# ethz-asl/laser_slam

Measured on AMD Instinct MI355X. Metric: scans_per_sec, higher is better.
Workload: dtype f32

## Files before the change

### laser_slam_amd/csrc/lsgpu_icp.hip

```cpp
#include <atomic>
#include <cstring>
#include <cmath>
#include <cstdio>
#include <cstdlib>
#include <string>
#include <vector>
#include <chrono>
#include <system_error>
#include <thread>
#include <type_traits>
#include <utility>

#include <dlfcn.h>

#include <hip/hip_runtime.h>
#include <rccl/rccl.h>

#include "../../include/lsgpu_icp.h"
#include "lsgpu_grid.hip.h"
#include "lsgpu_tuning.h"
#include "lsgpu_policy.h"
#include "lsgpu_knn.hip.h"
#include "lsgpu_knn_k.hip.h"
#include "lsgpu_snf.hip.h"
// ... 1781 lines not shown
      std::vector<uint32_t> sizes{(uint32_t)n}, next;
      h->gs_lvl_first.clear(); h->gs_lvl_blocks.clear();
      uint32_t rows = 0, segs = 0;
      for (int L = 0; L < glevels; ++L) {
        uint32_t fb = 0;
        next.clear();
        for (uint32_t c : sizes) {
          fb += (c + kGsTile - 1u) / kGsTile;
          next.push_back(c - c / 2u); next.push_back(c / 2u);
        }
        h->gs_lvl_first.push_back(rows); h->gs_lvl_blocks.push_back(fb);
        rows += fb; segs += (uint32_t)sizes.size();
        sizes.swap(next);
      }
      HIPC(h->gs_tab.reserve(rows)); HIPC(h->gs_sblk.reserve(segs));
      if (glevels <= kGsPlanLevels && ((size_t)1 << (glevels - 1)) <= kGsPlanSegs) {
        GsPlanArgs pa{};
        for (int L = 0; L < glevels; ++L) pa.first[L] = h->gs_lvl_first[L];
        hipLaunchKernelGGL(k_gs_plan, dim3(glevels), dim3(1024), 0, h->stream, (uint32_t)n, pa, h->gs_tab.p, h->gs_sblk.p);
        HIPC(hipGetLastError());
      } else {
        std::vector<GsBlock> tab;
        std::vector<GsSegBlocks> sblk;
        std::vector<std::pair<uint32_t, uint32_t>> segsz{{0u, (uint32_t)n}};
        for (int L = 0; L < glevels; ++L) {
          uint32_t fb = 0;
          std::vector<std::pair<uint32_t, uint32_t>> nx;
          for (uint32_t sidx = 0; sidx < segsz.size(); ++sidx) {
            const uint32_t st = segsz[sidx].first, c = segsz[sidx].second;
            const uint32_t nb = (c + kGsTile - 1u) / kGsTile;
            sblk.push_back(GsSegBlocks{fb, nb, st, c});
            for (uint32_t k = 0; k < nb; ++k)
              tab.push_back(GsBlock{st + k * kGsTile, std::min(kGsTile, c - k * kGsTile), sidx, st, c, fb, nb, 0u});
            fb += nb;
            const uint32_t left = c - c / 2u;
            nx.push_back({st, left}); nx.push_back({st + left, c - left});
          }
          segsz.swap(nx);
        }
        HIPC(hipMemcpyAsync(h->gs_tab.p, tab.data(), tab.size() * sizeof(GsBlock), hipMemcpyHostToDevice, h->stream));
        HIPC(hipMemcpyAsync(h->gs_sblk.p, sblk.data(), sblk.size() * sizeof(GsSegBlocks), hipMemcpyHostToDevice, h->stream));
        HIPC(hipStreamSynchronize(h->stream));
      }
      h->gs_plan_n = n; h->gs_plan_levels = glevels;
    }
    const size_t nseg_g = (size_t)1 << glevels;
    int cap = 1;
    for (uint32_t v : h->gs_lvl_blocks) cap = std::max(cap, (int)v);
    for (auto& bf : h->gs_e) HIPC(bf.reserve(n));
    for (auto& bf : h->gs_k) HIPC(bf.reserve(n));
    HIPC(h->gs_hist.reserve(4 * 256 * (nseg_g + 1))); HIPC(h->gs_median.reserve(nseg_g)); HIPC(h->gs_cand_n.reserve(2 * nseg_g + 2));
    const size_t cand_room = std::max<size_t>(nseg_g / 2, 1) * kGsCandRoom;
    HIPC(h->gs_cand.reserve(cand_room)); HIPC(h->gs_cand_blk.reserve(cand_room));
    HIPC(h->gs_cl.reserve((size_t)2 * cap)); HIPC(h->gs_err.reserve(8)); HIPC(h->gs_rng.reserve(2 * nseg_g + 2));
    HIPC(h->ssn_axis_a.reserve(nseg_g)); HIPC(h->ssn_axis_b.reserve(nseg_g));
    uint32_t* cand_n[2] = {h->gs_cand_n.p, h->gs_cand_n.p + nseg_g + 1};
    uint32_t* sig_cur = reinterpret_cast<uint32_t*>(h->ssn_axis_a.p);
    uint32_t* sig_nxt = reinterpret_cast<uint32_t*>(h->ssn_axis_b.p);
    GsSet in, out;
    in.e = h->gs_e[0].p; out.e = h->gs_e[1].p;
    for (int d = 0; d < 3; ++d) { in.k[d] = h->gs_k[d].p; out.k[d] = h->gs_k[3 + d].p; }
    uint2* rng_cur = h->gs_rng.p;
    uint2* rng_nxt = h->gs_rng.p + nseg_g + 1;
    uint32_t* gh1[2] = {h->gs_hist.p, h->gs_hist.p + 256 * (nseg_g + 1)};
    uint32_t* gh2[2] = {h->gs_hist.p + 2 * 256 * (nseg_g + 1), h->gs_hist.p + 3 * 256 * (nseg_g + 1)};
    hipLaunchKernelGGL(k_gs_init, dim3(nblk(n)), dim3(256), 0, h->stream, src, (int)n, in, out.e, (const SsnSeg*)cur, (const uint32_t*)h->ssn_bb.p, rng_cur,
                       gh1[0], gh2[0], cand_n[0], sig_cur, h->gs_err.p);
    for (int L = 0; L < glevels; ++L) {
      const int ns = 1 << L, nb = (int)h->gs_lvl_blocks[L], par = L & 1;
      const GsBlock* tab = h->gs_tab.p + h->gs_lvl_first[L];
      const GsSegBlocks* sblk = h->gs_sblk.p + (ns - 1);
      hipLaunchKernelGGL(k_gs_hist<1>, dim3(nb), dim3(256), 0, h->stream, tab, cur, (const uint2*)rng_cur, in, gh1[par], gh2[par], h->gs_err.p);
      hipLaunchKernelGGL(k_gs_hist<2>, dim3(nb), dim3(256), 0, h->stream, tab, cur, (const uint2*)rng_cur, in, gh1[par], gh2[par], h->gs_err.p);
      const uint32_t lvl_cap = (uint32_t)std::min<size_t>(cand_room / (size_t)ns, (size_t)1 << 22);
      hipLaunchKernelGGL(k_gs_collect, dim3(nb), dim3(256), 0, h->stream, tab, cur, (const uint2*)rng_cur, (const uint32_t*)sig_cur, in,
                         (const uint32_t*)gh1[par], (const uint32_t*)gh2[par], cand_n[par], h->gs_cand.p, h->gs_cand_blk.p, lvl_cap, h->gs_cl.p);
      hipLaunchKernelGGL(k_gs_select, dim3(ns), dim3(L < 3 ? 1024 : 256), 0, h->stream, sblk, src, cur, (const uint32_t*)sig_cur, gh1[par], gh2[par],
                         gh1[par ^ 1], gh2[par ^ 1], cand_n[par], (const GsMedian*)h->gs_cand.p, (const uint32_t*)h->gs_cand_blk.p, lvl_cap, h->gs_cl.p,
                         h->gs_cl.p + cap, h->gs_median.p, nxt, sig_nxt, cand_n[par ^ 1], rng_nxt, h->gs_err.p);
      hipLaunchKernelGGL(k_gs_part, dim3(nb), dim3(kGsPartThreads), 0, h->stream, tab, cur, (const uint32_t*)sig_cur, in, out,
                         (const GsMedian*)h->gs_median.p, (const uint32_t*)(h->gs_cl.p + cap), (const SsnSeg*)nxt, rng_nxt, h->gs_err.p);
      std::swap(in, out);
      std::swap(cur, nxt);
      std::swap(sig_cur, sig_nxt);
      std::swap(rng_cur, rng_nxt);
    }
    idx = in.e;
    root_sig = sig_cur;
    HIPC(hipGetLastError());
  } else if (glevels > 0) {
    const size_t nseg_g = (size_t)1 << glevels;
    const int cap = (int)(n / kSegTile + (int64_t)(nseg_g / 2) + 2);
    HIPC(h->lane.scratch->vals_alt.reserve(n));
    HIPC(h->ssn_axis_a.reserve(nseg_g)); HIPC(h->ssn_axis_b.reserve(nseg_g)); HIPC(h->ssn_seg_fb.reserve(nseg_g));
    HIPC(h->ssn_blocktab.reserve((size_t)cap)); HIPC(h->lane.scratch->sort_hist.reserve((size_t)256 * cap + 256 + 4));
    uint32_t* keyA = reinterpret_cast<uint32_t*>(h->lane.scratch->keys.p);
    uint32_t* keyB = keyA + n;
    uint32_t* valA = h->lane.scratch->vals.p;
    uint32_t* valB = h->lane.scratch->vals_alt.p;
    uint32_t* bh = h->lane.scratch->sort_hist.p;
    uint32_t* dtot = bh + (size_t)256 * cap;
    uint32_t* nblocks_dev = dtot + 256;
    int* ax_cur = h->ssn_axis_a.p;
    int* ax_nxt = h->ssn_axis_b.p;
    HIPC(hipMemsetAsync(ax_cur, 0xFF, sizeof(int), h->stream));
    for (int L = 0; L < glevels; ++L) {
      const int ns = 1 << L;
      const int grid = (int)std::min<int64_t>(cap, n / kSegTile + ns + 1);
      hipLaunchKernelGGL(k_ssn_plan, dim3(1), dim3(256), 0, h->stream, cur, ns, knn, ax_cur, h->ssn_seg_fb.p,
                         h->ssn_blocktab.p, nblocks_dev);
      hipLaunchKernelGGL(k_ssn_keys32, dim3(nblk(n)), dim3(256), 0, h->stream, src, (int)n, valA, h->ssn_seg_of.p, cur,
                         h->ssn_seg_fb.p, L == 0 ? 1 : 0, keyA);
      for (int pass = 0; pass < 4; ++pass) {
        const uint32_t* kin = (pass & 1) ? keyB : keyA; const uint32_t* vin = (pass & 1) ? valB : valA;
        uint32_t* kout = (pass & 1) ? keyA : keyB; uint32_t* vout = (pass & 1) ? valA : valB;
        hipLaunchKernelGGL(k_seg_hist<kSegItems>, dim3(grid), dim3(256), 0, h->stream, kin, h->ssn_blocktab.p, nblocks_dev, 8 * pass, bh, cap);
        hipLaunchKernelGGL(k_seg_scan, dim3(256), dim3(256), 0, h->stream, bh, cap, nblocks_dev, dtot);
        hipLaunchKernelGGL((k_seg_scatter<kSegItems>), dim3(grid), dim3(256), 0, h->stream, kin, vin, kout, vout,
                           h->ssn_blocktab.p, nblocks_dev, 8 * pass, bh, dtot, cap);
      }
      idx = valA;
      hipLaunchKernelGGL(k_ssn_split, dim3(nblk(ns)), dim3(256), 0, h->stream, src, idx, cur, ns, knn, nxt, (const int*)ax_cur, ax_nxt);
      hipLaunchKernelGGL(k_ssn_assign, dim3(nblk(n)), dim3(256), 0, h->stream, (int)n, cur, knn, h->ssn_seg_of.p, L == 0 ? 1 : 0);
      std::swap(cur, nxt);
      std::swap(ax_cur, ax_nxt);
    }
    root_axis = ax_cur;
    HIPC(hipGetLastError());
  }
  if (glevels < levels) {
    if (glevels == 0) {
      hipLaunchKernelGGL(k_ssn_keys, dim3(nblk(n)), dim3(256), 0, h->stream, src, (int)n, (const uint32_t*)nullptr,
                         (const uint32_t*)nullptr, cur, knn, h->lane.scratch->keys.p, h->lane.scratch->vals.p);
      idx = h->lane.scratch->vals.p;
    }
    uint32_t* idx_rw = const_cast<uint32_t*>(idx);
    if (root_max == 8192)
      hipLaunchKernelGGL(k_ssn_tree<8192>, dim3(1 << glevels), dim3(1024), 0, h->stream, src, idx_rw, cur, knn, levels - glevels, h->ssn_seg_of.p, nxt, root_axis, root_sig);
// ... 1793 lines not shown
```

### laser_slam_amd/csrc/lsgpu_ssn_select.hip.h

```cpp
#pragma once
#include "lsgpu_ssn.hip.h"
#include "lsgpu_ssn_tree.hip.h"

namespace lsgpu {

#ifdef LSGPU_KNN_STATS
#define LSGPU_SEL_T(n) do { if (gridDim.x == 1 && threadIdx.x == 0) g_tree_dbg[n] = (unsigned long long)clock64(); } while (0)
#else
#define LSGPU_SEL_T(n) do { } while (0)
#endif

constexpr uint32_t kGsTile = 2048u;
constexpr int kGsPartThreads = 512;
constexpr uint32_t kGsCandCap = 2048u;
constexpr uint32_t kGsCandRoom = 16384u;
constexpr uint32_t kGsNoAxis = 0xFFu;
constexpr uint32_t kGsSelBlocks = 8192u;

struct GsSet {
  uint32_t* e;
  uint32_t* k[3];
};
__device__ __forceinline__ uint32_t* gs_k(const GsSet& g, int d) { return d == 0 ? g.k[0] : d == 1 ? g.k[1] : g.k[2]; }

// ... 19 lines not shown
  if (o1 == a) { x1 = o2; x2 = o3; }
  else { x1 = o1; x2 = o2 == a ? o3 : o2; }
}
__device__ __forceinline__ bool gs_less(uint32_t ka, uint32_t k1, uint32_t k2, uint32_t e, const GsMedian& m) {
  return ka != m.ka ? ka < m.ka : k1 != m.k1 ? k1 < m.k1 : k2 != m.k2 ? k2 < m.k2 : e < m.e;
}

constexpr int kGsPlanLevels = 24;
constexpr uint32_t kGsPlanSegs = 8192u;
struct GsPlanArgs { uint32_t first[kGsPlanLevels]; };
__global__ __launch_bounds__(1024) void k_gs_plan(uint32_t n, GsPlanArgs lvl, GsBlock* __restrict__ tab, GsSegBlocks* __restrict__ sblk) {
  __shared__ uint32_t fbs[kGsPlanSegs + 1];
  __shared__ uint2 sc[kGsPlanSegs];
  __shared__ uint32_t wsum[16], carry_sh;
  const uint32_t L = blockIdx.x, ns = 1u << L;
  const int lane = threadIdx.x & 63, w = threadIdx.x >> 6;
  if (threadIdx.x == 0) carry_sh = 0u;
  __syncthreads();
  for (uint32_t s0 = 0; s0 < ns; s0 += 1024u) {
    const uint32_t sg = s0 + threadIdx.x;
    uint32_t st = 0u, c = n;
    for (int bit = (int)L - 1; bit >= 0; --bit) {
      const uint32_t left = c - c / 2u;
      if ((sg >> bit) & 1u) { st += left; c -= left; } else c = left;
    }
    const uint32_t nb = sg < ns ? (c + kGsTile - 1u) / kGsTile : 0u;
    const uint32_t incl = wave_scan_incl_u32(nb, lane);
    if (lane == 63) wsum[w] = incl;
    __syncthreads();
    uint32_t before = carry_sh;
    for (int ww = 0; ww < w; ++ww) before += wsum[ww];
    if (sg < ns) { fbs[sg] = before + incl - nb; sc[sg] = make_uint2(st, c); }
    __syncthreads();
    if (threadIdx.x == 1023) carry_sh = before + incl;
    __syncthreads();
  }
  if (threadIdx.x == 0) fbs[ns] = carry_sh;
  __syncthreads();
  const uint32_t total = fbs[ns];
  for (uint32_t sg = threadIdx.x; sg < ns; sg += 1024u)
    sblk[(ns - 1u) + sg] = GsSegBlocks{fbs[sg], fbs[sg + 1u] - fbs[sg], sc[sg].x, sc[sg].y};
  GsBlock* __restrict__ t = tab + lvl.first[L];
  for (uint32_t j = threadIdx.x; j < total; j += 1024u) {
    uint32_t lo = 0u, hi = ns;
    while (hi - lo > 1u) { const uint32_t mid = (lo + hi) >> 1; if (fbs[mid] <= j) lo = mid; else hi = mid; }
    const uint32_t k = j - fbs[lo], st = sc[lo].x, c = sc[lo].y;
    const uint32_t off = k * kGsTile;
    t[j] = GsBlock{st + off, min(kGsTile, c - off), lo, st, c, fbs[lo], fbs[lo + 1u] - fbs[lo], 0u};
  }
}

__global__ __launch_bounds__(256) void k_gs_init(const float4* __restrict__ p, int n, GsSet out, uint32_t* __restrict__ other_e,
                                                 const SsnSeg* __restrict__ root, const uint32_t* __restrict__ bb,
                                                 uint2* __restrict__ rng, uint32_t* __restrict__ gh1_root,
                                                 uint32_t* __restrict__ gh2_root, uint32_t* __restrict__ cand_n_root,
                                                 uint32_t* __restrict__ sig_root, uint32_t* __restrict__ err) {
  const int i = blockIdx.x * 256 + threadIdx.x;
  if (blockIdx.x == 0) {
    gh1_root[threadIdx.x] = 0u; gh2_root[threadIdx.x] = 0u;
    if (threadIdx.x < 8) err[threadIdx.x] = 0u;
    if (threadIdx.x == 0) {
      const int a = ssn_cut_axis(root[0]); rng[0] = make_uint2(bb[a], bb[3 + a]);
      cand_n_root[0] = 0u; sig_root[0] = 0xFFFFFFFFu;
    }
  }
  if (i >= n) return;
  const float4 v = p[i];
  out.e[i] = (uint32_t)i; other_e[i] = (uint32_t)i;
  out.k[0][i] = float_order_key(v.x); out.k[1][i] = float_order_key(v.y); out.k[2][i] = float_order_key(v.z);
}

struct GsCut { int a; uint32_t klo, khi; float xlo, scale; };
__device__ __forceinline__ GsCut gs_cut(const SsnSeg& sg, const uint2 rng ) {
  GsCut c;
  c.a = ssn_cut_axis(sg);
  c.klo = rng.x; c.khi = rng.y >= rng.x ? rng.y : rng.x;
  c.xlo = float_from_order_key(c.klo);
  const float ext = float_from_order_key(c.khi) - c.xlo;
  c.scale = ext > 0.f ? 65536.0f / ext : 0.f;
  return c;
}
__device__ __forceinline__ uint32_t gs_bin16(const GsCut& c, uint32_t k) {
  const float t = (float_from_order_key(k) - c.xlo) * c.scale;
  return (uint32_t)fminf(fmaxf(t, 0.f), 65535.f);
}

__device__ __forceinline__ void gs_find_bin(const uint32_t* __restrict__ gh, uint32_t target, uint32_t* sh ,
                                            uint32_t& bin, uint32_t& below) {
  const int lane = threadIdx.x & 63, w = threadIdx.x >> 6;
  const bool act = threadIdx.x < 256u;
  const uint32_t tot = act ? gh[threadIdx.x] : 0u;
  const uint32_t incl = wave_scan_incl_u32(tot, lane);
  if (threadIdx.x == 0) { sh[4] = 0xFFFFFFFFu; sh[5] = 0u; }
  if (act && lane == 63) sh[w] = incl;
  __syncthreads();
  uint32_t before = 0u;
  for (int ww = 0; ww < w && ww < 4; ++ww) before += sh[ww];
  const uint32_t excl = before + incl - tot;
  if (act && tot != 0u && excl <= target && target < excl + tot) { sh[4] = threadIdx.x; sh[5] = excl; }
  __syncthreads();
  bin = sh[4]; below = sh[5];
  __syncthreads();
}

template <int PASS>
__global__ __launch_bounds__(256) void k_gs_hist(const GsBlock* __restrict__ tab, const SsnSeg* __restrict__ segs,
                                                 const uint2* __restrict__ rng, GsSet in, uint32_t* __restrict__ gh1,
                                                 uint32_t* __restrict__ gh2, uint32_t* __restrict__ err) {
  __shared__ uint32_t hist[256];
  __shared__ uint32_t sh[8];
  hist[threadIdx.x] = 0u;
  const GsBlock sb = tab[blockIdx.x];
  const GsCut c = gs_cut(segs[sb.seg], rng[sb.seg]);
  const uint32_t* __restrict__ ka = gs_k(in, c.a);
  uint32_t mb1 = 0u, below1 = 0u;
// ... 22 lines not shown
                                                    uint32_t* __restrict__ cl) {
  __shared__ uint32_t ws[4];
  __shared__ uint32_t sh[8];
  const GsBlock sb = tab[blockIdx.x];
  const GsCut c = gs_cut(segs[sb.seg], rng[sb.seg]);
  const uint32_t leftn = sb.seg_count - sb.seg_count / 2u;
  uint32_t mb1, below1, mb2, below2;
  gs_find_bin(gh1 + (size_t)sb.seg * 256u, leftn, sh, mb1, below1);
  gs_find_bin(gh2 + (size_t)sb.seg * 256u, leftn - below1, sh, mb2, below2);
  uint32_t x1, x2;
  gs_other_axes(sig[sb.seg], (uint32_t)c.a, x1, x2);
  const uint32_t* __restrict__ ka = gs_k(in, c.a);
  uint32_t left = 0u;
  const int lane = threadIdx.x & 63;
  for (uint32_t j0 = 0; j0 < sb.count; j0 += 256u) {
    const uint32_t j = j0 + threadIdx.x;
    const bool live = j < sb.count;
    const uint32_t i = sb.first + (live ? j : 0u);
    const uint32_t k = live ? ka[i] : 0u;
    const uint32_t b16 = gs_bin16(c, k), b1 = b16 >> 8, b2 = b16 & 255u;
    const bool is_cand = live && b1 == mb1 && b2 == mb2;
    if (live && (b1 < mb1 || (b1 == mb1 && b2 < mb2))) ++left;
    const unsigned long long m = __ballot(is_cand);
    if (m != 0ull) {
      uint32_t base = 0u;
      if (lane == 0) base = atomicAdd(&cand_n[sb.seg], (uint32_t)__popcll(m));
      base = (uint32_t)__shfl((int)base, 0);
      const uint32_t slot = base + (uint32_t)__popcll(m & ((1ull << lane) - 1ull));
      if (is_cand && slot < cap) {
        GsMedian md;
        md.ka = k; md.e = in.e[i];
        md.k1 = x1 != kGsNoAxis ? gs_k(in, (int)x1)[i] : 0u;
        md.k2 = x2 != kGsNoAxis ? gs_k(in, (int)x2)[i] : 0u;
        cand[(size_t)sb.seg * cap + slot] = md;
        cand_blk[(size_t)sb.seg * cap + slot] = blockIdx.x;
      }
    }
  }
  left = wave_sum_u32(left);
  if ((threadIdx.x & 63) == 0) ws[threadIdx.x >> 6] = left;
  __syncthreads();
  if (threadIdx.x == 0) cl[blockIdx.x] = ws[0] + ws[1] + ws[2] + ws[3];
}

__global__ __launch_bounds__(1024) void k_gs_select(const GsSegBlocks* __restrict__ sblk, const float4* __restrict__ p,
                                                   const SsnSeg* __restrict__ segs, const uint32_t* __restrict__ sig,
                                                   uint32_t* __restrict__ gh1, uint32_t* __restrict__ gh2,
                                                   uint32_t* __restrict__ gh1_next, uint32_t* __restrict__ gh2_next,
                                                   uint32_t* __restrict__ cand_n,
                                                   const GsMedian* __restrict__ cand, const uint32_t* __restrict__ cand_blk, uint32_t cap,
                                                   uint32_t* __restrict__ cl, uint32_t* __restrict__ clp, GsMedian* __restrict__ median,
                                                   SsnSeg* __restrict__ out, uint32_t* __restrict__ sig_out,
                                                   uint32_t* __restrict__ cand_n_next, uint2* __restrict__ rng_next,
                                                   uint32_t* __restrict__ err) {
  __shared__ GsMedian lc[kGsCandCap];
  __shared__ uint32_t med_slot;
  __shared__ GsMedian med_sh;
  __shared__ uint32_t sh[8];
  __shared__ uint32_t rh[256];
  __shared__ uint32_t lcnt[kGsSelBlocks];
  __shared__ uint32_t lblk[kGsCandCap];
  LSGPU_SEL_T(48);
  const uint32_t s = blockIdx.x;
  const GsSegBlocks q = sblk[s];
  const uint32_t n = cand_n[s];
  const uint32_t left = q.count - q.count / 2u;
  uint32_t mb1, below1, mb2, below2;
  gs_find_bin(gh1 + (size_t)s * 256u, left, sh, mb1, below1);
  gs_find_bin(gh2 + (size_t)s * 256u, left - below1, sh, mb2, below2);
  const uint32_t target = left - below1 - below2;
  LSGPU_SEL_T(49);
  if (threadIdx.x < 256u) {
    gh1_next[(size_t)(2u * s) * 256u + threadIdx.x] = 0u; gh1_next[(size_t)(2u * s + 1u) * 256u + threadIdx.x] = 0u;
    gh2_next[(size_t)(2u * s) * 256u + threadIdx.x] = 0u; gh2_next[(size_t)(2u * s + 1u) * 256u + threadIdx.x] = 0u;
  }
  if (threadIdx.x == 0) {
    med_slot = 0xFFFFFFFFu;
    cand_n_next[2u * s] = 0u; cand_n_next[2u * s + 1u] = 0u;
    rng_next[2u * s] = make_uint2(0xFFFFFFFFu, 0u); rng_next[2u * s + 1u] = make_uint2(0xFFFFFFFFu, 0u);
    if (n > cap || target >= n || mb1 == 0xFFFFFFFFu || mb2 == 0xFFFFFFFFu) { err[0] = 1u; err[1] = 3u; err[2] = s; err[3] = n; err[4] = target; }
  }
  const uint32_t c = min(n, cap);
  const GsMedian* __restrict__ gc = cand + (size_t)s * cap;
  const uint32_t* __restrict__ gb = cand_blk + (size_t)s * cap;
  const bool in_lds = c <= kGsCandCap;
  const bool lds_counts = q.nb <= kGsSelBlocks;
  if (lds_counts) for (uint32_t b = threadIdx.x; b < q.nb; b += blockDim.x) lcnt[b] = 0u;
  if (in_lds) for (uint32_t i = threadIdx.x; i < c; i += blockDim.x) { lc[i] = gc[i]; lblk[i] = gb[i]; }
  __syncthreads();
  LSGPU_SEL_T(50);
#ifdef LSGPU_KNN_STATS
  if (gridDim.x == 1 && threadIdx.x == 0) g_tree_dbg[54] = c;
#endif
  uint32_t arrived = 0u;
  if (c <= 256u) {
    const int lane = threadIdx.x & 63;
    const uint32_t w = threadIdx.x >> 6, nw = blockDim.x >> 6;
    GsMedian oj[4];
#pragma unroll
    for (int ch = 0; ch < 4; ++ch) {
      const uint32_t j = (uint32_t)(ch * 64 + lane);
      oj[ch] = j < c ? lc[j] : GsMedian{0xFFFFFFFFu, 0xFFFFFFFFu, 0xFFFFFFFFu, 0xFFFFFFFFu};
    }
    for (uint32_t i = w; i < c; i += nw) {
      const GsMedian me = lc[i];
      uint32_t r = 0u;
#pragma unroll
      for (int ch = 0; ch < 4; ++ch)
        if ((uint32_t)(ch * 64) < c) r += (uint32_t)__popcll(__ballot(gs_less(oj[ch].ka, oj[ch].k1, oj[ch].k2, oj[ch].e, me)));
      if (lane == 0) {
        if (r < target) {
          const uint32_t blk = lblk[i];
          if (lds_counts) atomicAdd(&lcnt[blk - q.fb], 1u); else arrived ^= atomicAdd(&cl[blk], 1u);
        }
        if (r == target) { med_slot = i; med_sh = me; }
      }
    }
  } else {
    GsMedian ch{0u, 0u, 0u, 0u};
    uint32_t rem = target;
    bool found = false;
    for (int pass = 0; pass < 16 && !found; ++pass) {
      const int field = pass >> 2, shift = 24 - 8 * (pass & 3);
      const uint32_t himask = shift == 24 ? 0u : 0xFFFFFFFFu << (shift + 8);
      if (threadIdx.x < 256u) rh[threadIdx.x] = 0u;
      __syncthreads();
      for (uint32_t i = threadIdx.x; i < c; i += blockDim.x) {
        const GsMedian o = in_lds ? lc[i] : gc[i];
        const bool before_ok = (field < 1 || o.ka == ch.ka) && (field < 2 || o.k1 == ch.k1) && (field < 3 || o.k2 == ch.k2);
        const uint32_t f = field == 0 ? o.ka : field == 1 ? o.k1 : field == 2 ? o.k2 : o.e;
        const uint32_t cf = field == 0 ? ch.ka : field == 1 ? ch.k1 : field == 2 ? ch.k2 : ch.e;
        if (before_ok && ((f ^ cf) & himask) == 0u) atomicAdd(&rh[(f >> shift) & 255u], 1u);
// ... 18 lines not shown
      }
      __syncthreads();
    }
    if (med_slot != 0xFFFFFFFFu) {
      const GsMedian m = med_sh;
      for (uint32_t i = threadIdx.x; i < c; i += blockDim.x) {
        const GsMedian o = in_lds ? lc[i] : gc[i];
        if (gs_less(o.ka, o.k1, o.k2, o.e, m)) {
          const uint32_t blk = in_lds ? lblk[i] : gb[i];
          if (lds_counts) atomicAdd(&lcnt[blk - q.fb], 1u); else arrived ^= atomicAdd(&cl[blk], 1u);
        }
      }
    }
  }
  asm volatile("" ::"v"(arrived));
  __syncthreads();
  LSGPU_SEL_T(51);
  {
    const int lane = threadIdx.x & 63, w = threadIdx.x >> 6;
    const bool act = threadIdx.x < 256u;
    uint32_t carry = 0u;
    for (uint32_t b0 = 0; b0 < q.nb; b0 += 256u) {
      const uint32_t b = b0 + threadIdx.x;
      const uint32_t v = act && b < q.nb ? (lds_counts ? cl[q.fb + b] + lcnt[b] : __hip_atomic_load(&cl[q.fb + b], __ATOMIC_RELAXED, __HIP_MEMORY_SCOPE_AGENT)) : 0u;
      const uint32_t incl = wave_scan_incl_u32(v, lane);
      if (act && lane == 63) sh[w] = incl;
      __syncthreads();
      uint32_t before = carry;
      for (int ww = 0; ww < w && ww < 4; ++ww) before += sh[ww];
      if (act && b < q.nb) clp[q.fb + b] = before + incl - v;
      carry += sh[0] + sh[1] + sh[2] + sh[3];
      __syncthreads();
    }
  }
  LSGPU_SEL_T(52);
  if (threadIdx.x == 0) {
    const bool have = med_slot != 0xFFFFFFFFu;
    const GsMedian m = have ? med_sh : GsMedian{0u, 0u, 0u, 0u};
    median[s] = m;
    const SsnSeg sg = segs[s];
    const int cut = ssn_cut_axis(sg);
    SsnSeg a = sg, b = sg;
    const float cutval = have ? coord_of(p[m.e], cut) : coord_of(make_float4(sg.hi[0], sg.hi[1], sg.hi[2], 0.f), cut);
#pragma unroll
    for (int d = 0; d < 3; ++d) {
      a.hi[d] = d == cut ? cutval : a.hi[d];
      b.lo[d] = d == cut ? cutval : b.lo[d];
    }
    a.start = q.start; a.count = left;
    b.start = q.start + left; b.count = q.count - left;
    out[2u * s] = a; out[2u * s + 1u] = b;
    const uint32_t sv = gs_sig_push(sig[s], (uint32_t)cut);
    sig_out[2u * s] = sv; sig_out[2u * s + 1u] = sv;
  }
  LSGPU_SEL_T(53);
}

__global__ __launch_bounds__(kGsPartThreads) void k_gs_part(const GsBlock* __restrict__ tab, const SsnSeg* __restrict__ segs,
                                                 const uint32_t* __restrict__ sig, GsSet in, GsSet out,
                                                 const GsMedian* __restrict__ median, const uint32_t* __restrict__ clp,
                                                 const SsnSeg* __restrict__ segs_next, uint2* __restrict__ rng_next,
                                                 uint32_t* __restrict__ err) {
  constexpr int kW = kGsPartThreads / 64, kI = (int)kGsTile / kGsPartThreads;
  __shared__ uint32_t ws[kW];
  __shared__ uint32_t rr[kW][4];
  __shared__ uint32_t stage[4][kGsTile];
  const int lane = threadIdx.x & 63, w = threadIdx.x >> 6;
  const GsBlock sb = tab[blockIdx.x];
  const SsnSeg sg = segs[sb.seg];
  const int a = ssn_cut_axis(sg);
  uint32_t x1, x2;
  gs_other_axes(sig[sb.seg], (uint32_t)a, x1, x2);
  const GsMedian m = median[sb.seg];
  const uint32_t base_left = clp[blockIdx.x];
  const uint32_t left_total = sb.seg_count - sb.seg_count / 2u;
  const uint32_t base_right = (sb.first - sb.seg_start) - base_left;
  uint32_t ev[kI], kx[kI], ky[kI], kz[kI], xl[kI];
  uint32_t carry = 0u;
  const int aL = ssn_cut_axis(segs_next[2u * sb.seg]), aR = ssn_cut_axis(segs_next[2u * sb.seg + 1u]);
  uint32_t mnL = 0xFFFFFFFFu, mxL = 0u, mnR = 0xFFFFFFFFu, mxR = 0u;
#pragma unroll
  for (int k = 0; k < kI; ++k) {
    const uint32_t j = (uint32_t)(w * (64 * kI) + k * 64 + lane);
    uint32_t v = 0u;
    ev[k] = kx[k] = ky[k] = kz[k] = 0u;
    if (j < sb.count) {
      const uint32_t i = sb.first + j;
      ev[k] = in.e[i]; kx[k] = in.k[0][i]; ky[k] = in.k[1][i]; kz[k] = in.k[2][i];
      const uint32_t ka = a == 0 ? kx[k] : a == 1 ? ky[k] : kz[k];
      const uint32_t k1 = x1 == kGsNoAxis ? 0u : x1 == 0u ? kx[k] : x1 == 1u ? ky[k] : kz[k];
      const uint32_t k2 = x2 == kGsNoAxis ? 0u : x2 == 0u ? kx[k] : x2 == 1u ? ky[k] : kz[k];
      v = gs_less(ka, k1, k2, ev[k], m) ? 1u : 0u;
      if (v) { const uint32_t kc = aL == 0 ? kx[k] : aL == 1 ? ky[k] : kz[k]; mnL = min(mnL, kc); mxL = max(mxL, kc); }
      else   { const uint32_t kc = aR == 0 ? kx[k] : aR == 1 ? ky[k] : kz[k]; mnR = min(mnR, kc); mxR = max(mxR, kc); }
    }
    const uint32_t incl = tree_wave_scan(v, lane);
    xl[k] = ((carry + incl - v) << 1) | v;
    carry += rl_u(incl, 63);
  }
  __syncthreads();
  mnL = ~wave_max_u32(~mnL); mxL = wave_max_u32(mxL); mnR = ~wave_max_u32(~mnR); mxR = wave_max_u32(mxR);
  if (lane == 0) { ws[w] = carry; rr[w][0] = mnL; rr[w][1] = mxL; rr[w][2] = mnR; rr[w][3] = mxR; }
  __syncthreads();
  if (threadIdx.x < 4) {
    const int q = (int)threadIdx.x;
    const bool is_min = (q & 1) == 0;
    uint32_t v = rr[0][q];
    for (int ww = 1; ww < kW; ++ww) v = is_min ? min(v, rr[ww][q]) : max(v, rr[ww][q]);
    uint32_t* word = reinterpret_cast<uint32_t*>(&rng_next[2u * sb.seg + (uint32_t)(q >> 1)]) + (q & 1);
    const uint32_t seen = __hip_atomic_load(word, __ATOMIC_RELAXED, __HIP_MEMORY_SCOPE_AGENT);
    if (is_min ? v < seen : v > seen) { if (is_min) atomicMin(word, v); else atomicMax(word, v); }
  }
  uint32_t before = 0u;
  for (int ww = 0; ww < w; ++ww) before += ws[ww];
  uint32_t nleft = 0u;
  for (int ww = 0; ww < kW; ++ww) nleft += ws[ww];
#pragma unroll
  for (int k = 0; k < kI; ++k) {
    const uint32_t j = (uint32_t)(w * (64 * kI) + k * 64 + lane);
    if (j < sb.count) {
      const uint32_t lbefore = before + (xl[k] >> 1);
      const uint32_t slot = (xl[k] & 1u) ? lbefore : nleft + (j - lbefore);
      stage[0][slot] = ev[k]; stage[1][slot] = kx[k]; stage[2][slot] = ky[k]; stage[3][slot] = kz[k];
    }
  }
  __syncthreads();
  const uint32_t dst_left = sb.seg_start + base_left, dst_right = sb.seg_start + left_total + base_right;
  const uint32_t pos0 = sb.first - sb.seg_start;
  const bool bad = base_left > pos0 || base_left + nleft > left_total ||
                   (pos0 - base_left) + (sb.count - nleft) > sb.seg_count - left_total;
  if (bad) {
    if (threadIdx.x == 0) { err[0] = 1u; err[5] = 4u; err[6] = sb.seg; err[7] = dst_left; }
    for (uint32_t t = threadIdx.x; t < sb.count; t += (uint32_t)kGsPartThreads) {
      const uint32_t d = sb.first + t;
      out.e[d] = stage[0][t]; out.k[0][d] = stage[1][t]; out.k[1][d] = stage[2][t]; out.k[2][d] = stage[3][t];
    }
    return;
  }
#pragma unroll
  for (int k = 0; k < kI; ++k) {
    const uint32_t t = (uint32_t)(k * kGsPartThreads) + threadIdx.x;
    if (t < sb.count) {
      const uint32_t d = t < nleft ? dst_left + t : dst_right + (t - nleft);
      out.e[d] = stage[0][t]; out.k[0][d] = stage[1][t]; out.k[1][d] = stage[2][t]; out.k[2][d] = stage[3][t];
    }
  }
}

}
```

### laser_slam_amd/csrc/lsgpu_tuning.h

```cpp

#pragma once
#include <cstdio>
#include <cstdlib>
#include <cstring>

extern char** environ;

namespace lsgpu {

struct Tuning {
  int query_order = -1;
  float q_elev = 0.f, q_sect = 0.f;
  float gap = 0.002f;
  int chunk_budget = 512, chunk_budget_wide = 1024;
  int wide_iters = 3;
  float route_r = 0.02f;
  int route_chunks = 1024;
  int route_heavy_max = 1024;
  int route_dense = 512;
  bool predict_select = true, commit_select = true, comm_commit = true, seed_cap = true;
  int sel_amb_cap = 256;
  bool two_pass_select = true;
  bool short_last_group = true;
  bool fused_select = true;
  bool lazy_need = true;
  bool lane_split = true;
  bool lookahead = true;
  bool index_rest = true;
  bool side_stream = true;
  int front_guess = 2048;
  int sort_items = 0;
  bool ssn_sort_levels = false;
  int ssn_root = 0;
  int ne_blocks = 256;
  bool split_update = false;
  double comm_timeout_ms = 30000.0;
  int knn_dbg = 0;
  bool cone = true;
  bool cone_probe = true;
  int cone_rows = 128, cone_cols = 8192, cone_from = 2;
  float cone_max_occupancy = 7.0f;
  float cone_heavy_steps = 1024.f;
  float cone_heavy_share = 0.07f;
};

namespace tuning_detail {
inline bool flag(const char* name) { return getenv(name) != nullptr; }
inline double number(const char* name, double def, double lo, double hi) {
  const char* e = getenv(name);
  if (!e) return def;
  char* end = nullptr;
  const double v = strtod(e, &end);
  if (end == e || *end != '\0' || !(v >= lo && v <= hi)) {
    fprintf(stderr, "liblsgpu_icp: %s=%s is not a number in [%g, %g]; using the default %g\n", name, e, lo, hi, def);
    return def;
  }
  return v;
}
inline Tuning read() {
  Tuning t;
  t.query_order = (int)number("LSGPU_QUERY_ORDER", -1, -1, 1);
  t.q_elev = (float)number("LSGPU_Q_ELEV", 0, 0, 45);
  t.q_sect = (float)number("LSGPU_Q_SECT", 0, 0, 45);
  t.gap = (float)number("LSGPU_GAP", 0.002, 0, 1);
  t.chunk_budget = (int)number("LSGPU_BUDGET", 512, 1, 1 << 20);
  t.chunk_budget_wide = (int)number("LSGPU_BUDGET_WIDE", 1024, 1, 1 << 20);
  t.wide_iters = (int)number("LSGPU_WIDE_ITERS", 3, 0, 1 << 20);
  t.route_r = (float)number("LSGPU_ROUTE_R", 0.02, 1e-6, 1e6);
  t.route_chunks = (int)number("LSGPU_ROUTE_CHUNKS", 1024, 1, 1 << 30);
  t.route_heavy_max = (int)number("LSGPU_ROUTE_HEAVY_MAX", 1024, -1, 1 << 30);
  t.route_dense = (int)number("LSGPU_ROUTE_DENSE", 512, 1, 1 << 30);
  t.split_update = flag("LSGPU_SPLIT_UPDATE");
  t.predict_select = !flag("LSGPU_NO_PREDICT") && !t.split_update;
  t.commit_select = !flag("LSGPU_NO_COMMIT");
  t.fused_select = !flag("LSGPU_NO_FUSED_SELECT");
  t.short_last_group = !flag("LSGPU_FULL_GROUPS");
  t.two_pass_select = !flag("LSGPU_THREE_PASS_SELECT");
  t.sel_amb_cap = (int)number("LSGPU_SEL_AMB_CAP", 256, 0, 256);
  t.comm_commit = !flag("LSGPU_NO_COMM_COMMIT");
  t.seed_cap = !flag("LSGPU_NO_SEED_CAP");
  t.lazy_need = !flag("LSGPU_NO_LAZY");
  t.lane_split = !flag("LSGPU_NO_SPLIT");
  t.side_stream = !flag("LSGPU_NO_SIDE_STREAM");
  t.lookahead = !flag("LSGPU_NO_LOOKAHEAD");
  t.index_rest = !flag("LSGPU_NO_INDEX_REST");
  t.front_guess = (int)number("LSGPU_FRONT_GUESS", 2048, 0, 8192);
  t.sort_items = (int)number("LSGPU_SORT_ITEMS", 0, 0, 16);
  if (t.sort_items != 0 && t.sort_items != 4 && t.sort_items != 8 && t.sort_items != 16) {
    fprintf(stderr, "liblsgpu_icp: LSGPU_SORT_ITEMS must be 4, 8 or 16; choosing by size\n");
    t.sort_items = 0;
  }
  t.ssn_sort_levels = flag("LSGPU_SSN_SORT_LEVELS");
  t.ssn_root = (int)number("LSGPU_SSN_ROOT", 0, 0, 8192);
  if (t.ssn_root != 0 && t.ssn_root != 2048 && t.ssn_root != 4096 && t.ssn_root != 8192) {
    fprintf(stderr, "liblsgpu_icp: LSGPU_SSN_ROOT must be 2048, 4096 or 8192; choosing by size\n");
    t.ssn_root = 0;
  }
  t.ne_blocks = (int)number("LSGPU_NE_BLOCKS", 256, 64, 2048);
  t.comm_timeout_ms = number("LSGPU_COMM_TIMEOUT_MS", 30000, 1, 1e9);
  t.knn_dbg = (int)number("LSGPU_KNN_DBG", 0, 0, 1 << 20);
  t.cone = !flag("LSGPU_NO_CONE");
  t.cone_probe = !flag("LSGPU_NO_CONE_PROBE");
  t.cone_from = (int)number("LSGPU_CONE_FROM", 2, 1, 1 << 20);
  t.cone_max_occupancy = (float)number("LSGPU_CONE_MAX_OCC", 7.0, 0.0, 1e9);
  t.cone_heavy_steps = (float)number("LSGPU_CONE_HEAVY_STEPS", 1024.0, 0.0, 1e9);
  t.cone_heavy_share = (float)number("LSGPU_CONE_HEAVY_SHARE", 0.07, 0.0, 2.0);
  t.cone_rows = (int)number("LSGPU_CONE_ROWS", 128, 8, 1024);
  t.cone_cols = (int)number("LSGPU_CONE_COLS", 8192, 64, 65536) & ~3;
  static const char* known[] = {"LSGPU_QUERY_ORDER", "LSGPU_Q_ELEV", "LSGPU_Q_SECT", "LSGPU_GAP", "LSGPU_BUDGET", "LSGPU_BUDGET_WIDE", "LSGPU_WIDE_ITERS",
                                "LSGPU_ROUTE_R", "LSGPU_ROUTE_CHUNKS", "LSGPU_ROUTE_HEAVY_MAX", "LSGPU_ROUTE_DENSE", "LSGPU_SPLIT_UPDATE", "LSGPU_NO_PREDICT", "LSGPU_NO_COMMIT",
                                "LSGPU_NO_COMM_COMMIT", "LSGPU_NO_SEED_CAP", "LSGPU_NO_LAZY", "LSGPU_NO_SPLIT", "LSGPU_NO_SIDE_STREAM", "LSGPU_NO_LOOKAHEAD", "LSGPU_NO_INDEX_REST", "LSGPU_CELLS_SPLIT", "LSGPU_NO_FUSED_SELECT", "LSGPU_FULL_GROUPS", "LSGPU_THREE_PASS_SELECT", "LSGPU_SEL_AMB_CAP", "LSGPU_FRONT_GUESS",
                                "LSGPU_SORT_ITEMS", "LSGPU_SSN_ROOT", "LSGPU_SSN_SORT_LEVELS",
                                "LSGPU_NE_BLOCKS", "LSGPU_COMM_TIMEOUT_MS", "LSGPU_KNN_DBG", "LSGPU_NO_CONE", "LSGPU_NO_CONE_PROBE", "LSGPU_CONE_ROWS", "LSGPU_CONE_COLS", "LSGPU_CONE_FROM", "LSGPU_CONE_MAX_OCC", "LSGPU_CONE_HEAVY_STEPS", "LSGPU_CONE_HEAVY_SHARE",
                                "LSGPU_SO", "LSGPU_STATS_SO", "LSGPU_BATCH_POOLS", "LSGPU_BATCH_UNIQ", "LSGPU_GS_DEBUG", "LSGPU_GOLDEN_DIR", "LSGPU_SEQ_PERTURB", "LSGPU_SEQ_POSES", "LSGPU_TEST_INPUT_FILTERS",
                                nullptr};
  for (char** e = environ; e && *e; ++e) {
    if (strncmp(*e, "LSGPU_", 6) != 0) continue;
    const char* eq = strchr(*e, '=');
    const size_t len = eq ? (size_t)(eq - *e) : strlen(*e);
    bool ok = false;
    for (const char** k = known; *k; ++k) ok = ok || (strlen(*k) == len && strncmp(*k, *e, len) == 0);
    if (!ok) fprintf(stderr, "liblsgpu_icp: unknown switch %.*s ignored (see csrc/lsgpu_tuning.h)\n", (int)len, *e);
  }
  return t;
}
}

inline const Tuning& tuning() {
  static const Tuning t = tuning_detail::read();
  return t;
}

}
```

Measured before the change: 253.2.

## Fuse next-level coarse histogram and child ranges into partition kernel

The partition kernel now builds the first-pass coarse histogram for both child segments in shared memory and tracks per-axis min/max for all three axes. This lets later levels skip the separate k_gs_hist<1> launch and its full read of the keys. Child cut ranges are then derived in the select kernel from the three-axis ranges and the median. The cost is extra shared-memory atomics and registers in the partition kernel, and a larger range buffer. The old path stays available behind LSGPU_GS_HIST_PASS.

```diff
diff --git a/laser_slam_amd/csrc/lsgpu_icp.hip b/laser_slam_amd/csrc/lsgpu_icp.hip
--- a/laser_slam_amd/csrc/lsgpu_icp.hip
+++ b/laser_slam_amd/csrc/lsgpu_icp.hip
@@ -1857,7 +1857,7 @@
     HIPC(h->gs_hist.reserve(4 * 256 * (nseg_g + 1))); HIPC(h->gs_median.reserve(nseg_g)); HIPC(h->gs_cand_n.reserve(2 * nseg_g + 2));
     const size_t cand_room = std::max<size_t>(nseg_g / 2, 1) * kGsCandRoom;
     HIPC(h->gs_cand.reserve(cand_room)); HIPC(h->gs_cand_blk.reserve(cand_room));
-    HIPC(h->gs_cl.reserve((size_t)2 * cap)); HIPC(h->gs_err.reserve(8)); HIPC(h->gs_rng.reserve(2 * nseg_g + 2));
+    HIPC(h->gs_cl.reserve((size_t)2 * cap)); HIPC(h->gs_err.reserve(8)); HIPC(h->gs_rng.reserve(8 * (nseg_g + 1)));
     HIPC(h->ssn_axis_a.reserve(nseg_g)); HIPC(h->ssn_axis_b.reserve(nseg_g));
     uint32_t* cand_n[2] = {h->gs_cand_n.p, h->gs_cand_n.p + nseg_g + 1};
     uint32_t* sig_cur = reinterpret_cast<uint32_t*>(h->ssn_axis_a.p);
@@ -1869,26 +1869,37 @@
     uint2* rng_nxt = h->gs_rng.p + nseg_g + 1;
     uint32_t* gh1[2] = {h->gs_hist.p, h->gs_hist.p + 256 * (nseg_g + 1)};
     uint32_t* gh2[2] = {h->gs_hist.p + 2 * 256 * (nseg_g + 1), h->gs_hist.p + 3 * 256 * (nseg_g + 1)};
+    const bool part_hist = !tuning().gs_hist_pass;
+    uint2* rng3_cur = part_hist ? h->gs_rng.p + 2 * (nseg_g + 1) : nullptr;
+    uint2* rng3_nxt = part_hist ? h->gs_rng.p + 5 * (nseg_g + 1) : nullptr;
     hipLaunchKernelGGL(k_gs_init, dim3(nblk(n)), dim3(256), 0, h->stream, src, (int)n, in, out.e, (const SsnSeg*)cur, (const uint32_t*)h->ssn_bb.p, rng_cur,
-                       gh1[0], gh2[0], cand_n[0], sig_cur, h->gs_err.p);
+                       rng3_cur, gh1[0], gh2[0], cand_n[0], sig_cur, h->gs_err.p);
     for (int L = 0; L < glevels; ++L) {
       const int ns = 1 << L, nb = (int)h->gs_lvl_blocks[L], par = L & 1;
       const GsBlock* tab = h->gs_tab.p + h->gs_lvl_first[L];
       const GsSegBlocks* sblk = h->gs_sblk.p + (ns - 1);
-      hipLaunchKernelGGL(k_gs_hist<1>, dim3(nb), dim3(256), 0, h->stream, tab, cur, (const uint2*)rng_cur, in, gh1[par], gh2[par], h->gs_err.p);
+      if (!part_hist || L == 0)
+        hipLaunchKernelGGL(k_gs_hist<1>, dim3(nb), dim3(256), 0, h->stream, tab, cur, (const uint2*)rng_cur, in, gh1[par], gh2[par], h->gs_err.p);
       hipLaunchKernelGGL(k_gs_hist<2>, dim3(nb), dim3(256), 0, h->stream, tab, cur, (const uint2*)rng_cur, in, gh1[par], gh2[par], h->gs_err.p);
       const uint32_t lvl_cap = (uint32_t)std::min<size_t>(cand_room / (size_t)ns, (size_t)1 << 22);
       hipLaunchKernelGGL(k_gs_collect, dim3(nb), dim3(256), 0, h->stream, tab, cur, (const uint2*)rng_cur, (const uint32_t*)sig_cur, in,
                          (const uint32_t*)gh1[par], (const uint32_t*)gh2[par], cand_n[par], h->gs_cand.p, h->gs_cand_blk.p, lvl_cap, h->gs_cl.p);
       hipLaunchKernelGGL(k_gs_select, dim3(ns), dim3(L < 3 ? 1024 : 256), 0, h->stream, sblk, src, cur, (const uint32_t*)sig_cur, gh1[par], gh2[par],
                          gh1[par ^ 1], gh2[par ^ 1], cand_n[par], (const GsMedian*)h->gs_cand.p, (const uint32_t*)h->gs_cand_blk.p, lvl_cap, h->gs_cl.p,
-                         h->gs_cl.p + cap, h->gs_median.p, nxt, sig_nxt, cand_n[par ^ 1], rng_nxt, h->gs_err.p);
-      hipLaunchKernelGGL(k_gs_part, dim3(nb), dim3(kGsPartThreads), 0, h->stream, tab, cur, (const uint32_t*)sig_cur, in, out,
-                         (const GsMedian*)h->gs_median.p, (const uint32_t*)(h->gs_cl.p + cap), (const SsnSeg*)nxt, rng_nxt, h->gs_err.p);
+                         h->gs_cl.p + cap, h->gs_median.p, nxt, sig_nxt, cand_n[par ^ 1], rng_nxt, (const uint2*)rng3_cur, rng3_nxt, h->gs_err.p);
+      if (part_hist)
+        hipLaunchKernelGGL(k_gs_part<true>, dim3(nb), dim3(kGsPartThreads), 0, h->stream, tab, cur, (const uint32_t*)sig_cur, in, out,
+                           (const GsMedian*)h->gs_median.p, (const uint32_t*)(h->gs_cl.p + cap), (const SsnSeg*)nxt, rng_nxt, rng3_nxt, gh1[par ^ 1],
+                           L + 1 < glevels ? 1 : 0, h->gs_err.p);
+      else
+        hipLaunchKernelGGL(k_gs_part<false>, dim3(nb), dim3(kGsPartThreads), 0, h->stream, tab, cur, (const uint32_t*)sig_cur, in, out,
+                           (const GsMedian*)h->gs_median.p, (const uint32_t*)(h->gs_cl.p + cap), (const SsnSeg*)nxt, rng_nxt, (uint2*)nullptr,
+                           (uint32_t*)nullptr, 0, h->gs_err.p);
       std::swap(in, out);
       std::swap(cur, nxt);
       std::swap(sig_cur, sig_nxt);
       std::swap(rng_cur, rng_nxt);
+      std::swap(rng3_cur, rng3_nxt);
     }
     idx = in.e;
     root_sig = sig_cur;
diff --git a/laser_slam_amd/csrc/lsgpu_ssn_select.hip.h b/laser_slam_amd/csrc/lsgpu_ssn_select.hip.h
--- a/laser_slam_amd/csrc/lsgpu_ssn_select.hip.h
+++ b/laser_slam_amd/csrc/lsgpu_ssn_select.hip.h
@@ -95,7 +95,8 @@
 
 __global__ __launch_bounds__(256) void k_gs_init(const float4* __restrict__ p, int n, GsSet out, uint32_t* __restrict__ other_e,
                                                  const SsnSeg* __restrict__ root, const uint32_t* __restrict__ bb,
-                                                 uint2* __restrict__ rng, uint32_t* __restrict__ gh1_root,
+                                                 uint2* __restrict__ rng, uint2* __restrict__ rng3_root ,
+                                                 uint32_t* __restrict__ gh1_root,
                                                  uint32_t* __restrict__ gh2_root, uint32_t* __restrict__ cand_n_root,
                                                  uint32_t* __restrict__ sig_root, uint32_t* __restrict__ err) {
   const int i = blockIdx.x * 256 + threadIdx.x;
@@ -104,6 +105,7 @@
     if (threadIdx.x < 8) err[threadIdx.x] = 0u;
     if (threadIdx.x == 0) {
       const int a = ssn_cut_axis(root[0]); rng[0] = make_uint2(bb[a], bb[3 + a]);
+      if (rng3_root) for (int d = 0; d < 3; ++d) rng3_root[d] = make_uint2(bb[d], bb[3 + d]);
       cand_n_root[0] = 0u; sig_root[0] = 0xFFFFFFFFu;
     }
   }
@@ -232,7 +234,8 @@
                                                    uint32_t* __restrict__ cl, uint32_t* __restrict__ clp, GsMedian* __restrict__ median,
                                                    SsnSeg* __restrict__ out, uint32_t* __restrict__ sig_out,
                                                    uint32_t* __restrict__ cand_n_next, uint2* __restrict__ rng_next,
-                                                   uint32_t* __restrict__ err) {
+                                                   const uint2* __restrict__ rng3 ,
+                                                   uint2* __restrict__ rng3_next, uint32_t* __restrict__ err) {
   __shared__ GsMedian lc[kGsCandCap];
   __shared__ uint32_t med_slot;
   __shared__ GsMedian med_sh;
@@ -244,6 +247,8 @@
   const uint32_t s = blockIdx.x;
   const GsSegBlocks q = sblk[s];
   const uint32_t n = cand_n[s];
+  uint2 r0 = make_uint2(0u, 0u), r1 = r0, r2 = r0;
+  if (rng3) { r0 = rng3[3u * s]; r1 = rng3[3u * s + 1u]; r2 = rng3[3u * s + 2u]; }
   const uint32_t left = q.count - q.count / 2u;
   uint32_t mb1, below1, mb2, below2;
   gs_find_bin(gh1 + (size_t)s * 256u, left, sh, mb1, below1);
@@ -257,7 +262,7 @@
   if (threadIdx.x == 0) {
     med_slot = 0xFFFFFFFFu;
     cand_n_next[2u * s] = 0u; cand_n_next[2u * s + 1u] = 0u;
-    rng_next[2u * s] = make_uint2(0xFFFFFFFFu, 0u); rng_next[2u * s + 1u] = make_uint2(0xFFFFFFFFu, 0u);
+    if (!rng3) { rng_next[2u * s] = make_uint2(0xFFFFFFFFu, 0u); rng_next[2u * s + 1u] = make_uint2(0xFFFFFFFFu, 0u); }
     if (n > cap || target >= n || mb1 == 0xFFFFFFFFu || mb2 == 0xFFFFFFFFu) { err[0] = 1u; err[1] = 3u; err[2] = s; err[3] = n; err[4] = target; }
   }
   const uint32_t c = min(n, cap);
@@ -382,19 +387,32 @@
     out[2u * s] = a; out[2u * s + 1u] = b;
     const uint32_t sv = gs_sig_push(sig[s], (uint32_t)cut);
     sig_out[2u * s] = sv; sig_out[2u * s + 1u] = sv;
+    if (rng3) {
+      const int ca = ssn_cut_axis(a), cb = ssn_cut_axis(b);
+      uint2 ra = ca == 0 ? r0 : ca == 1 ? r1 : r2, rb = cb == 0 ? r0 : cb == 1 ? r1 : r2;
+      if (have && ca == cut) ra.y = m.ka;
+      if (have && cb == cut) rb.x = m.ka;
+      rng_next[2u * s] = ra; rng_next[2u * s + 1u] = rb;
+#pragma unroll
+      for (uint32_t d = 0; d < 6u; ++d) rng3_next[6u * s + d] = make_uint2(0xFFFFFFFFu, 0u);
+    }
   }
   LSGPU_SEL_T(53);
 }
 
+template <bool HIST>
 __global__ __launch_bounds__(kGsPartThreads) void k_gs_part(const GsBlock* __restrict__ tab, const SsnSeg* __restrict__ segs,
                                                  const uint32_t* __restrict__ sig, GsSet in, GsSet out,
                                                  const GsMedian* __restrict__ median, const uint32_t* __restrict__ clp,
                                                  const SsnSeg* __restrict__ segs_next, uint2* __restrict__ rng_next,
+                                                 uint2* __restrict__ rng3_next, uint32_t* __restrict__ gh1_next, int more,
                                                  uint32_t* __restrict__ err) {
   constexpr int kW = kGsPartThreads / 64, kI = (int)kGsTile / kGsPartThreads;
+  constexpr int kR = HIST ? 12 : 4;
   __shared__ uint32_t ws[kW];
-  __shared__ uint32_t rr[kW][4];
+  __shared__ uint32_t rr[kW][kR];
   __shared__ uint32_t stage[4][kGsTile];
+  __shared__ uint32_t hist[HIST ? 512 : 1];
   const int lane = threadIdx.x & 63, w = threadIdx.x >> 6;
   const GsBlock sb = tab[blockIdx.x];
   const SsnSeg sg = segs[sb.seg];
@@ -409,37 +427,75 @@
   uint32_t carry = 0u;
   const int aL = ssn_cut_axis(segs_next[2u * sb.seg]), aR = ssn_cut_axis(segs_next[2u * sb.seg + 1u]);
   uint32_t mnL = 0xFFFFFFFFu, mxL = 0u, mnR = 0xFFFFFFFFu, mxR = 0u;
+  uint32_t mn3[6] = {0xFFFFFFFFu, 0xFFFFFFFFu, 0xFFFFFFFFu, 0xFFFFFFFFu, 0xFFFFFFFFu, 0xFFFFFFFFu}, mx3[6] = {0u, 0u, 0u, 0u, 0u, 0u};
+  const bool fill = HIST && more != 0;
+  GsCut cL{}, cR{};
+  if (fill) {
+    cL = gs_cut(segs_next[2u * sb.seg], rng_next[2u * sb.seg]);
+    cR = gs_cut(segs_next[2u * sb.seg + 1u], rng_next[2u * sb.seg + 1u]);
+    for (uint32_t t = threadIdx.x; t < 512u; t += (uint32_t)kGsPartThreads) hist[t] = 0u;
+    __syncthreads();
+  }
 #pragma unroll
   for (int k = 0; k < kI; ++k) {
     const uint32_t j = (uint32_t)(w * (64 * kI) + k * 64 + lane);
     uint32_t v = 0u;
-    ev[k] = kx[k] = ky[k] = kz[k] = 0u;
+    uint32_t ce = 0u, cx = 0u, cy = 0u, cz = 0u;
     if (j < sb.count) {
       const uint32_t i = sb.first + j;
-      ev[k] = in.e[i]; kx[k] = in.k[0][i]; ky[k] = in.k[1][i]; kz[k] = in.k[2][i];
-      const uint32_t ka = a == 0 ? kx[k] : a == 1 ? ky[k] : kz[k];
-      const uint32_t k1 = x1 == kGsNoAxis ? 0u : x1 == 0u ? kx[k] : x1 == 1u ? ky[k] : kz[k];
-      const uint32_t k2 = x2 == kGsNoAxis ? 0u : x2 == 0u ? kx[k] : x2 == 1u ? ky[k] : kz[k];
-      v = gs_less(ka, k1, k2, ev[k], m) ? 1u : 0u;
-      if (v) { const uint32_t kc = aL == 0 ? kx[k] : aL == 1 ? ky[k] : kz[k]; mnL = min(mnL, kc); mxL = max(mxL, kc); }
-      else   { const uint32_t kc = aR == 0 ? kx[k] : aR == 1 ? ky[k] : kz[k]; mnR = min(mnR, kc); mxR = max(mxR, kc); }
-    }
+      ce = in.e[i]; cx = in.k[0][i]; cy = in.k[1][i]; cz = in.k[2][i];
+      const uint32_t ka = a == 0 ? cx : a == 1 ? cy : cz;
+      const uint32_t k1 = x1 == kGsNoAxis ? 0u : x1 == 0u ? cx : x1 == 1u ? cy : cz;
+      const uint32_t k2 = x2 == kGsNoAxis ? 0u : x2 == 0u ? cx : x2 == 1u ? cy : cz;
+      v = gs_less(ka, k1, k2, ce, m) ? 1u : 0u;
+      const uint32_t kcL = aL == 0 ? cx : aL == 1 ? cy : cz, kcR = aR == 0 ? cx : aR == 1 ? cy : cz;
+      const uint32_t kc = v ? kcL : kcR;
+      if (!HIST) {
+        if (v) { mnL = min(mnL, kc); mxL = max(mxL, kc); } else { mnR = min(mnR, kc); mxR = max(mxR, kc); }
+      } else if (fill) {
+        GsCut cc;
+        cc.a = v ? aL : aR; cc.klo = v ? cL.klo : cR.klo; cc.khi = v ? cL.khi : cR.khi; cc.xlo = v ? cL.xlo : cR.xlo; cc.scale = v ? cL.scale : cR.scale;
+        atomicAdd(&hist[(v ? 0u : 256u) + (gs_bin16(cc, kc) >> 8)], 1u);
+        const uint32_t far = 0xFFFFFFFFu;
+        mn3[0] = min(mn3[0], v ? cx : far); mn3[1] = min(mn3[1], v ? cy : far); mn3[2] = min(mn3[2], v ? cz : far);
+        mn3[3] = min(mn3[3], v ? far : cx); mn3[4] = min(mn3[4], v ? far : cy); mn3[5] = min(mn3[5], v ? far : cz);
+        mx3[0] = max(mx3[0], v ? cx : 0u); mx3[1] = max(mx3[1], v ? cy : 0u); mx3[2] = max(mx3[2], v ? cz : 0u);
+        mx3[3] = max(mx3[3], v ? 0u : cx); mx3[4] = max(mx3[4], v ? 0u : cy); mx3[5] = max(mx3[5], v ? 0u : cz);
+      }
+    }
+    ev[k] = ce; kx[k] = cx; ky[k] = cy; kz[k] = cz;
     const uint32_t incl = tree_wave_scan(v, lane);
     xl[k] = ((carry + incl - v) << 1) | v;
     carry += rl_u(incl, 63);
   }
   __syncthreads();
-  mnL = ~wave_max_u32(~mnL); mxL = wave_max_u32(mxL); mnR = ~wave_max_u32(~mnR); mxR = wave_max_u32(mxR);
-  if (lane == 0) { ws[w] = carry; rr[w][0] = mnL; rr[w][1] = mxL; rr[w][2] = mnR; rr[w][3] = mxR; }
-  __syncthreads();
-  if (threadIdx.x < 4) {
+  if (!HIST) {
+    mnL = ~wave_max_u32(~mnL); mxL = wave_max_u32(mxL); mnR = ~wave_max_u32(~mnR); mxR = wave_max_u32(mxR);
+    if (lane == 0) { rr[w][0] = mnL; rr[w][1] = mxL; rr[w][2] = mnR; rr[w][3] = mxR; }
+  } else if (fill) {
+#pragma unroll
+    for (int q = 0; q < 6; ++q) {
+      const uint32_t lo = ~wave_max_u32(~mn3[q]), hi = wave_max_u32(mx3[q]);
+      if (lane == 0) { rr[w][2 * q] = lo; rr[w][2 * q + 1] = hi; }
+    }
+  }
+  if (lane == 0) ws[w] = carry;
+  __syncthreads();
+  if ((int)threadIdx.x < kR && (!HIST || fill)) {
     const int q = (int)threadIdx.x;
     const bool is_min = (q & 1) == 0;
     uint32_t v = rr[0][q];
     for (int ww = 1; ww < kW; ++ww) v = is_min ? min(v, rr[ww][q]) : max(v, rr[ww][q]);
-    uint32_t* word = reinterpret_cast<uint32_t*>(&rng_next[2u * sb.seg + (uint32_t)(q >> 1)]) + (q & 1);
+    uint2* pair = HIST ? &rng3_next[6u * sb.seg + (uint32_t)(q >> 1)] : &rng_next[2u * sb.seg + (uint32_t)(q >> 1)];
+    uint32_t* word = reinterpret_cast<uint32_t*>(pair) + (q & 1);
     const uint32_t seen = __hip_atomic_load(word, __ATOMIC_RELAXED, __HIP_MEMORY_SCOPE_AGENT);
     if (is_min ? v < seen : v > seen) { if (is_min) atomicMin(word, v); else atomicMax(word, v); }
+  }
+  if (fill) {
+    for (uint32_t t = threadIdx.x; t < 512u; t += (uint32_t)kGsPartThreads) {
+      const uint32_t v = hist[t];
+      if (v) atomicAdd(&gh1_next[(size_t)(2u * sb.seg + (t >> 8)) * 256u + (t & 255u)], v);
+    }
   }
   uint32_t before = 0u;
   for (int ww = 0; ww < w; ++ww) before += ws[ww];
diff --git a/laser_slam_amd/csrc/lsgpu_tuning.h b/laser_slam_amd/csrc/lsgpu_tuning.h
--- a/laser_slam_amd/csrc/lsgpu_tuning.h
+++ b/laser_slam_amd/csrc/lsgpu_tuning.h
@@ -32,6 +32,7 @@
   int sort_items = 0;
   bool ssn_sort_levels = false;
   int ssn_root = 0;
+  bool gs_hist_pass = false;
   int ne_blocks = 256;
   bool split_update = false;
   double comm_timeout_ms = 30000.0;
@@ -96,6 +97,7 @@
     fprintf(stderr, "liblsgpu_icp: LSGPU_SSN_ROOT must be 2048, 4096 or 8192; choosing by size\n");
     t.ssn_root = 0;
   }
+  t.gs_hist_pass = flag("LSGPU_GS_HIST_PASS");
   t.ne_blocks = (int)number("LSGPU_NE_BLOCKS", 256, 64, 2048);
   t.comm_timeout_ms = number("LSGPU_COMM_TIMEOUT_MS", 30000, 1, 1e9);
   t.knn_dbg = (int)number("LSGPU_KNN_DBG", 0, 0, 1 << 20);
@@ -110,7 +112,7 @@
   static const char* known[] = {"LSGPU_QUERY_ORDER", "LSGPU_Q_ELEV", "LSGPU_Q_SECT", "LSGPU_GAP", "LSGPU_BUDGET", "LSGPU_BUDGET_WIDE", "LSGPU_WIDE_ITERS",
                                 "LSGPU_ROUTE_R", "LSGPU_ROUTE_CHUNKS", "LSGPU_ROUTE_HEAVY_MAX", "LSGPU_ROUTE_DENSE", "LSGPU_SPLIT_UPDATE", "LSGPU_NO_PREDICT", "LSGPU_NO_COMMIT",
                                 "LSGPU_NO_COMM_COMMIT", "LSGPU_NO_SEED_CAP", "LSGPU_NO_LAZY", "LSGPU_NO_SPLIT", "LSGPU_NO_SIDE_STREAM", "LSGPU_NO_LOOKAHEAD", "LSGPU_NO_INDEX_REST", "LSGPU_CELLS_SPLIT", "LSGPU_NO_FUSED_SELECT", "LSGPU_FULL_GROUPS", "LSGPU_THREE_PASS_SELECT", "LSGPU_SEL_AMB_CAP", "LSGPU_FRONT_GUESS",
-                                "LSGPU_SORT_ITEMS", "LSGPU_SSN_ROOT", "LSGPU_SSN_SORT_LEVELS",
+                                "LSGPU_SORT_ITEMS", "LSGPU_SSN_ROOT", "LSGPU_SSN_SORT_LEVELS", "LSGPU_GS_HIST_PASS",
                                 "LSGPU_NE_BLOCKS", "LSGPU_COMM_TIMEOUT_MS", "LSGPU_KNN_DBG", "LSGPU_NO_CONE", "LSGPU_NO_CONE_PROBE", "LSGPU_CONE_ROWS", "LSGPU_CONE_COLS", "LSGPU_CONE_FROM", "LSGPU_CONE_MAX_OCC", "LSGPU_CONE_HEAVY_STEPS", "LSGPU_CONE_HEAVY_SHARE",
                                 "LSGPU_SO", "LSGPU_STATS_SO", "LSGPU_BATCH_POOLS", "LSGPU_BATCH_UNIQ", "LSGPU_GS_DEBUG", "LSGPU_GOLDEN_DIR", "LSGPU_SEQ_PERTURB", "LSGPU_SEQ_POSES", "LSGPU_TEST_INPUT_FILTERS",
                                 nullptr};
```

Result: no change. 252.5 (-0.3%).
